# brantburnett/Snappier

Hardware: AMD Instinct MI355X
Metric: uncompressed GB/s block compress+decompress, 64 KiB blocks (higher is better)
Workload: dtype u8

## Files before the change

### snappier_amd/csrc/compress_lanes.hip

```cpp
#include <cstdlib>

#include "snp_device.h"

#ifndef SNP_CL_FLAT
#define SNP_CL_FLAT 1
#endif
#ifndef SNP_CL_SLOTS
#define SNP_CL_SLOTS 1
#endif

namespace {

constexpr u32 kDefaultSlots = SNP_CL_SLOTS;

constexpr u32 crc_step32(u32 x)
{
    for (int k = 0; k < 32; ++k) x = (x >> 1) ^ ((x & 1u) ? 0x82F63B78u : 0u);
    return x;
}

__device__ __forceinline__ u32 check_bits(u32 bytes) { return (bytes * 0x9E3779B1u) & 0xffff0000u; }

__device__ __forceinline__ u32 table_swap(u32* p, u32 v) { return __hip_atomic_exchange(p, v, __ATOMIC_RELAXED, __HIP_MEMORY_SCOPE_AGENT); }

struct LaneCtx {
    const u8* src;
    u8* dst;
    u32* table;
    u32 first4;
    u32 n;
    u32 mask;
    u32 hmask;
};

template <int VARIANT>
__device__ __forceinline__ u32 lane_hash(const LaneCtx& c, u32 bytes, const u16 (*lut)[256])
{
    u32 hash;
    if constexpr (VARIANT == SNP_HASH_CRC32C) {
        hash = lut[0][bytes & 0xffu] ^ lut[1][(bytes >> 8) & 0xffu] ^ lut[2][(bytes >> 16) & 0xffu] ^ lut[3][bytes >> 24] ^ c.hmask;
    } else {
        hash = (0x1e35a7bdu * bytes) >> 17;
    }
    return (hash & c.mask) >> 1;
}

__device__ __forceinline__ u32 lane_emit_literal(const LaneCtx& c, u32 op, u32 s, u32 len)
{
    u8* o = c.dst + op;
    const u32 k = len - 1;
    u32 hdr;
    if (k < 60) { o[0] = static_cast<u8>(k << 2); hdr = 1; }
    else if (k < 256) { o[0] = static_cast<u8>(60u << 2); o[1] = static_cast<u8>(k); hdr = 2; }
    else { o[0] = static_cast<u8>(61u << 2); o[1] = static_cast<u8>(k); o[2] = static_cast<u8>(k >> 8); hdr = 3; }
    const u8* src = c.src + s;
    u8* d = o + hdr;
    u32 i = 0;
    for (; i + 16 <= len; i += 16)
        *reinterpret_cast<snp_u128_unaligned*>(d + i) = *reinterpret_cast<const snp_u128_unaligned*>(src + i);
    for (; i + 4 <= len; i += 4) st32u(d + i, ld32u(src + i));
    for (; i < len; ++i) d[i] = src[i];
    return op + hdr + len;
}

__device__ __forceinline__ u32 lane_emit_literal16(const LaneCtx& c, u32 op, u32 s, u32 len, const snp_u128_unaligned& first, u32 cap, bool merge)
{
    u8* o = c.dst + op;
    const u32 k = len - 1;
    if (merge && len <= 15 && op + 16 <= cap) {
        snp_u128_unaligned w;
        w.v[0] = (first.v[0] << 8) | (k << 2);
        w.v[1] = __builtin_amdgcn_alignbit(first.v[1], first.v[0], 24);
        w.v[2] = __builtin_amdgcn_alignbit(first.v[2], first.v[1], 24);
        w.v[3] = __builtin_amdgcn_alignbit(first.v[3], first.v[2], 24);
        *reinterpret_cast<snp_u128_unaligned*>(o) = w;
        return op + 1 + len;
    }
    u32 hdr;
    if (k < 60) { o[0] = static_cast<u8>(k << 2); hdr = 1; }
    else if (k < 256) { o[0] = static_cast<u8>(60u << 2); o[1] = static_cast<u8>(k); hdr = 2; }
    else { o[0] = static_cast<u8>(61u << 2); o[1] = static_cast<u8>(k); o[2] = static_cast<u8>(k >> 8); hdr = 3; }
    u8* d = o + hdr;
    if (len >= 16 || op + hdr + 16 <= cap) {
        *reinterpret_cast<snp_u128_unaligned*>(d) = first;
    } else {
        u32 w[4] = {first.v[0], first.v[1], first.v[2], first.v[3]};
        u32 at = 0, wi = 0;
        if (len & 8) { st32u(d, w[0]); st32u(d + 4, w[1]); at = 8; wi = 2; }
        if (len & 4) { st32u(d + at, w[wi]); at += 4; ++wi; }
        u32 rest = w[wi & 3];
        if (len & 2) { d[at] = static_cast<u8>(rest); d[at + 1] = static_cast<u8>(rest >> 8); rest >>= 16; at += 2; }
        if (len & 1) d[at] = static_cast<u8>(rest);
    }
    if (len > 16) {
        const u8* src = c.src + s;
        u32 i = 16;
        for (; i + 16 <= len; i += 16)
            *reinterpret_cast<snp_u128_unaligned*>(d + i) = *reinterpret_cast<const snp_u128_unaligned*>(src + i);
        if (i < len)
            *reinterpret_cast<snp_u128_unaligned*>(d + len - 16) = *reinterpret_cast<const snp_u128_unaligned*>(src + len - 16);
    }
    return op + hdr + len;
}

__device__ __forceinline__ u32 lane_emit_copy64(u8* dst, u32 op, u32 off, u32 len, u32 cap)
{
    u8* o = dst + op;
    const bool one = len < 12 && off < 2048;
    const u32 w = one ? (1u | ((len - 4) << 2) | ((off >> 8) << 5) | ((off & 0xffu) << 8)) : (2u | ((len - 1) << 2) | (off << 8));
    if (op + 4 <= cap) {
        st32u(o, w);
    } else {
        o[0] = static_cast<u8>(w);
        o[1] = static_cast<u8>(w >> 8);
        if (!one) o[2] = static_cast<u8>(w >> 16);
    }
    return op + (one ? 2u : 3u);
}

__device__ __forceinline__ u32 lane_emit_copy(u8* dst, u32 op, u32 off, u32 len, u32 cap = 0)
{
    while (len >= 68) { op = lane_emit_copy64(dst, op, off, 64, cap); len -= 64; }
    if (len > 64) { op = lane_emit_copy64(dst, op, off, 60, cap); len -= 60; }
    return lane_emit_copy64(dst, op, off, len, cap);
}

__device__ __forceinline__ u32 lane_find_match_length(const u8* src, u32 s1, u32 s2, u32 n)
{
    u32 matched = 0;
    while (s2 + matched + 8 <= n) {
        const u64 x = ld64u(src + s1 + matched) ^ ld64u(src + s2 + matched);
        if (x) return matched + (static_cast<u32>(__builtin_ctzll(x)) >> 3);
        matched += 8;
    }
    while (s2 + matched < n && src[s1 + matched] == src[s2 + matched]) ++matched;
    return matched;
}

constexpr u32 kStageStride = 100;

struct OutStage {
    u8* lds;
    u32 flushed;
};

__device__ __forceinline__ void stage_flush64(const LaneCtx& c, OutStage& st)
{
    u8* g = c.dst + st.flushed;
    typedef u32 v4u __attribute__((ext_vector_type(4), aligned(1)));
#pragma unroll
    for (u32 i = 0; i < 64; i += 16) {
        const snp_u128_unaligned q = *reinterpret_cast<const snp_u128_unaligned*>(st.lds + i);
        const v4u v = {q.v[0], q.v[1], q.v[2], q.v[3]};
        __builtin_nontemporal_store(v, reinterpret_cast<v4u*>(g + i));
    }
    const snp_u128_unaligned t0 = *reinterpret_cast<const snp_u128_unaligned*>(st.lds + 64);
    const snp_u128_unaligned t1 = *reinterpret_cast<const snp_u128_unaligned*>(st.lds + 80);
    *reinterpret_cast<snp_u128_unaligned*>(st.lds) = t0;
    *reinterpret_cast<snp_u128_unaligned*>(st.lds + 16) = t1;
    st.flushed += 64;
}

__device__ __forceinline__ void stage_drain(const LaneCtx& c, OutStage& st, u32 op)
{
    const u32 fill = op - st.flushed;
    u8* g = c.dst + st.flushed;
    u32 i = 0;
    for (; i + 16 <= fill; i += 16)
        *reinterpret_cast<snp_u128_unaligned*>(g + i) = *reinterpret_cast<const snp_u128_unaligned*>(st.lds + i);
    for (; i < fill; ++i) g[i] = st.lds[i];
    st.flushed = op;
}

enum : int {
    kOptBlindLiterals = 1,
    kOptBlindLiteral16 = 2,
    kOptBlindCopies = 4,
    kOptShortExtend = 8,
    kOptStagedOutput = 16,
    kOptExchangeProbe = 64,
    kOptInputWindow = 128,
};

template <int VARIANT, u32 kSlots, bool SMALL>
__global__ __launch_bounds__(SNP_WAVE) void k_compress_lanes(const u8* __restrict__ in, const u64* __restrict__ in_off,
                                                            const u32* __restrict__ in_len, u32 nblocks,
                                                            u8* __restrict__ out, const u64* __restrict__ out_off,
                                                            u32* __restrict__ out_len, i32* __restrict__ status,
                                                            int emit_varint, const snp_table_pieces tp, int opts,
                                                            const u32* __restrict__ max_len, u32 small_max)
{
    __shared__ u16 lut[4][256];
    if (VARIANT == SNP_HASH_CRC32C) {
        for (u32 e = threadIdx.x; e < 1024; e += blockDim.x)
            lut[e >> 8][e & 255u] = static_cast<u16>(crc_step32((e & 255u) << (8 * (e >> 8))) & 0x7ffeu);
        __syncthreads();
    }
    __shared__ u8 s_out[SMALL ? 16 : SNP_WAVE * kStageStride];
    const u32 b = blockIdx.x * blockDim.x + threadIdx.x;
    const u32 maxlen = *max_len;
    if (SMALL ? maxlen > small_max : (small_max != 0 && maxlen <= small_max)) return;
    extern __shared__ __attribute__((aligned(16))) u8 s_dyn[];
    const u32 tstride = maxlen > 16384 ? 16384u : maxlen < 256 ? 256u : (2u << (31u - __clz(maxlen - 1)));
    u32* wt;
    {
        const u32 first = blockIdx.x * blockDim.x;
        const u32 mine = nblocks - first < blockDim.x ? nblocks - first : blockDim.x;
        const u32 piece = first / tp.piece_frags;
        wt = tp.p[piece] + static_cast<size_t>(first - piece * tp.piece_frags) * tstride;
        const size_t words = static_cast<size_t>(mine) * tstride;
        if (tstride == 16384u) {
            typedef u32 v4u __attribute__((ext_vector_type(4)));
            const v4u zero4 = {0, 0, 0, 0};
            for (size_t i = static_cast<size_t>(threadIdx.x) * 4; i < words; i += static_cast<size_t>(blockDim.x) * 4)
                __builtin_nontemporal_store(zero4, reinterpret_cast<v4u*>(wt + i));
        } else {
            for (size_t i = static_cast<size_t>(threadIdx.x) * 4; i < words; i += static_cast<size_t>(blockDim.x) * 4)
                *reinterpret_cast<uint4*>(wt + i) = make_uint4(0, 0, 0, 0);
        }
        asm volatile("s_waitcnt vmcnt(0)" ::: "memory");
    }
    if (b >= nblocks) return;
    const bool staged = (opts & kOptStagedOutput) != 0;
    const bool t_swap = kSlots == 1 && (opts & kOptExchangeProbe) != 0;
    bool in_win = (opts & kOptInputWindow) != 0;
    OutStage stg{(SMALL ? s_dyn + blockDim.x * (small_max + 16u) : s_out) + threadIdx.x * kStageStride, 0};

    LaneCtx c;
    c.dst = out + out_off[b];
    c.n = in_len[b];
    c.table = wt + static_cast<size_t>(threadIdx.x) * tstride;
    const u32 n = c.n;
    if constexpr (SMALL) {
        const u8* g = in + in_off[b];
        u8* mine = s_dyn + threadIdx.x * (small_max + 16u);
        u32 i = 0;
        for (; i + 16 <= n; i += 16) {
            const snp_u128_unaligned q = *reinterpret_cast<const snp_u128_unaligned*>(g + i);
            *reinterpret_cast<uint4*>(mine + i) = make_uint4(q.v[0], q.v[1], q.v[2], q.v[3]);
        }
        for (; i + 4 <= n; i += 4) *reinterpret_cast<u32*>(mine + i) = ld32u(g + i);
        for (; i < n; ++i) mine[i] = g[i];
        c.src = mine;
    } else {
        c.src = in + in_off[b];
    }
    c.first4 = n >= 4 ? ld32u(c.src) : 0u;
    if (n > SNP_BLOCK_SIZE) { out_len[b] = 0; status[b] = SNP_ERR_BAD_ARG; return; }

    u32 op = 0;
    if (emit_varint) {
        u32 v = n;
        while (v >= 128) { c.dst[op++] = static_cast<u8>(v | 0x80u); v >>= 7; }
        c.dst[op++] = static_cast<u8>(v);
    }
    stg.flushed = op;

    u32 ip = 0;
#if SNP_CL_FLAT
    enum : u32 { kScan = 0, kPost = 1, kExtend = 2, kDone = 3 };
    u32 mode = kDone;
    u32 next_emit = 0, skip = 32, cand = 0, base = 0, mlen = 0, limit = 0;
    snp_u128_unaligned win = {};
    u32 win_at = 0x80000000u;
    in_win = in_win && n >= 32;
    if (n >= 15) {
        const u32 tsize = n > 16384 ? 16384u : n < 256 ? 256u : (2u << (31u - __clz(n - 1)));
        c.mask = 2 * (tsize - 1);
        c.hmask = static_cast<u16>(crc_step32(c.mask) & 0x7ffeu);
        limit = n - 15;
        mode = kScan;
        ip = 1;
    }
    const u32 lit_cap = (opts & kOptBlindLiterals) ? 32u + n + n / 6u : 0u;
    while (__any(mode != kDone)) {
        u32 cp_len = 0, cp_off = 0;
        u32 lit_len = 0;
        snp_u128_unaligned lit16 = {};
        const bool post = mode == kPost;
        const bool scanning = mode == kScan || post;
        u32 p[kSlots], nx[kSlots], sk[kSlots], d[kSlots], h[kSlots], cv[kSlots];
        bool legal[kSlots];
        u64 w0 = 0;
        if (scanning) {
            u32 q = ip, sv = skip;
            bool ok = true;
#pragma unroll
            for (u32 k = 0; k < kSlots; ++k) {
                const u32 bb = post ? 0u : sv >> 5;
                sv += bb;
                p[k] = q;
                nx[k] = q + bb;
                sk[k] = sv;
                ok = ok && (post ? k == 0 : nx[k] <= limit);
                legal[k] = ok;
                q = nx[k];
            }
            const u32 at = ip - (post ? 1u : 0u);
            if (in_win) {
                u32 o = at - win_at;
                if (o > 8u) {
                    win_at = min(at, n - 16u);
                    win = *reinterpret_cast<const snp_u128_unaligned*>(c.src + win_at);
                    o = at - win_at;
                }
                const u32 dq = o >> 2, sh = (o & 3u) * 8u;
                const u32 a0 = dq == 0 ? win.v[0] : dq == 1 ? win.v[1] : win.v[2];
                const u32 a1 = dq == 0 ? win.v[1] : dq == 1 ? win.v[2] : win.v[3];
                const u32 a2 = dq == 0 ? win.v[2] : dq == 1 ? win.v[3] : 0u;
                const u64 lo = (static_cast<u64>(a1) << 32) | a0;
                w0 = sh ? (lo >> sh) | (static_cast<u64>(a2) << (64u - sh)) : lo;
            } else {
                w0 = ld64u(c.src + at);
            }
        } else {
#pragma unroll
            for (u32 k = 0; k < kSlots; ++k) { p[k] = nx[k] = sk[k] = 0; legal[k] = false; }
        }
        const bool ext = mode == kExtend;
        const bool ext_wide = ext && base + mlen + 32 <= n;
        snp_u128_unaligned xa0 = {}, xa1 = {}, xb0 = {}, xb1 = {};
        if (ext_wide) {
            const u8* a = c.src + cand + mlen;
            const u8* bq = c.src + base + mlen;
            xa0 = *reinterpret_cast<const snp_u128_unaligned*>(a);
            xb0 = *reinterpret_cast<const snp_u128_unaligned*>(bq);
            if (!(opts & kOptShortExtend)) {
                xa1 = *reinterpret_cast<const snp_u128_unaligned*>(a + 16);
                xb1 = *reinterpret_cast<const snp_u128_unaligned*>(bq + 16);
            }
        }
        u32 hm1 = ~0u, vm1 = 0;
        bool swapped = false;
        if (scanning) {
            if (post) {
                const u32 dm1 = static_cast<u32>(w0);
                hm1 = lane_hash<VARIANT>(c, dm1, lut);
                vm1 = (ip - 1) | check_bits(dm1);
                if (tstride == 16384u) __builtin_nontemporal_store(vm1, &c.table[hm1]);
                else c.table[hm1] = vm1;
                d[0] = static_cast<u32>(w0 >> 8);
            } else {
                d[0] = static_cast<u32>(w0);
            }
#pragma unroll
            for (u32 k = 1; k < kSlots; ++k) {
                d[k] = 0;
                if (legal[k]) {
                    const u32 delta = p[k] - p[0];
                    d[k] = delta <= 4 ? static_cast<u32>(w0 >> (8 * delta)) : ld32u(c.src + p[k]);
                }
            }
#pragma unroll
            for (u32 k = 0; k < kSlots; ++k) h[k] = lane_hash<VARIANT>(c, d[k], lut);
            if (t_swap) {
                swapped = legal[0] && h[0] != hm1;
                cv[0] = !legal[0] ? 0u : swapped ? table_swap(&c.table[h[0]], p[0] | check_bits(d[0])) : vm1;
            } else {
#pragma unroll
                for (u32 k = 0; k < kSlots; ++k) cv[k] = legal[k] ? c.table[h[k]] : 0u;
            }
        }
        if (ext) {
            bool finished = false;
            if (ext_wide) {
                const u64 x0 = (static_cast<u64>(xa0.v[0] ^ xb0.v[0])) | (static_cast<u64>(xa0.v[1] ^ xb0.v[1]) << 32);
                const u64 x1 = (static_cast<u64>(xa0.v[2] ^ xb0.v[2])) | (static_cast<u64>(xa0.v[3] ^ xb0.v[3]) << 32);
                const u64 x2 = (static_cast<u64>(xa1.v[0] ^ xb1.v[0])) | (static_cast<u64>(xa1.v[1] ^ xb1.v[1]) << 32);
                const u64 x3 = (static_cast<u64>(xa1.v[2] ^ xb1.v[2])) | (static_cast<u64>(xa1.v[3] ^ xb1.v[3]) << 32);
                finished = true;
                if (x0) mlen += static_cast<u32>(__builtin_ctzll(x0)) >> 3;
                else if (x1) mlen += 8 + (static_cast<u32>(__builtin_ctzll(x1)) >> 3);
                else if (opts & kOptShortExtend) { mlen += 16; finished = false; }
                else if (x2) mlen += 16 + (static_cast<u32>(__builtin_ctzll(x2)) >> 3);
                else if (x3) mlen += 24 + (static_cast<u32>(__builtin_ctzll(x3)) >> 3);
                else { mlen += 32; finished = false; }
            } else {
                for (u32 k = 0; k < 4 && !finished; ++k) {
                    if (base + mlen + 8 <= n) {
                        const u64 x = ld64u(c.src + cand + mlen) ^ ld64u(c.src + base + mlen);
                        if (x) { mlen += static_cast<u32>(__builtin_ctzll(x)) >> 3; finished = true; }
                        else mlen += 8;
                    } else {
                        while (base + mlen < n && c.src[cand + mlen] == c.src[base + mlen]) ++mlen;
                        finished = true;
                    }
                }
            }
            if (finished) {
                ip = base + mlen;
                cp_len = mlen;
                cp_off = base - cand;
                mode = ip >= limit ? kDone : kPost;
            }
        }
        if (scanning) {
#pragma unroll
            for (u32 k = 1; k < kSlots; ++k)
#pragma unroll
                for (u32 i = 0; i < k; ++i)
                    if (legal[k] && h[i] == h[k]) cv[k] = p[i] | check_bits(d[i]);
            u32 kw = kSlots;
#pragma unroll
            for (u32 k = kSlots; k-- > 0;) {
                const u32 pos = cv[k] & 0xffffu;
                const bool want = legal[k] && (pos == 0 ? c.first4 == d[k] : (cv[k] & 0xffff0000u) == check_bits(d[k]));
                if (want) kw = k;
            }
            u32 wp = 0, wpos = 0;
#pragma unroll
            for (u32 k = 0; k < kSlots; ++k)
                if (kw == k) { wp = p[k]; wpos = cv[k] & 0xffffu; }
            snp_u128_unaligned cb = {}, pb = {}, lb = {};
            if (kw < kSlots) {
                cb = *reinterpret_cast<const snp_u128_unaligned*>(c.src + wpos);
                pb = *reinterpret_cast<const snp_u128_unaligned*>(c.src + wp);
                if (!post) lb = *reinterpret_cast<const snp_u128_unaligned*>(c.src + next_emit);
            }
            bool ended = false;
#pragma unroll
            for (u32 k = 0; k < kSlots; ++k) {
                if (!ended && k <= kw) {
                    if (!legal[k]) {
                        if (!post) { ended = true; ip = next_emit; mode = kDone; }
                    } else if (!swapped) {
                        c.table[h[k]] = p[k] | check_bits(d[k]);
                    }
                }
            }
            if (!ended) {
                bool hit = false;
                if (kw < kSlots) {
                    const u64 x0 = (static_cast<u64>(cb.v[0] ^ pb.v[0])) | (static_cast<u64>(cb.v[1] ^ pb.v[1]) << 32);
                    const u64 x1 = (static_cast<u64>(cb.v[2] ^ pb.v[2])) | (static_cast<u64>(cb.v[3] ^ pb.v[3]) << 32);
                    hit = static_cast<u32>(x0) == 0;
                    if (hit) {
                        if (!post) {
                            if (staged) { lit_len = wp - next_emit; lit16 = lb; }
                            else op = lane_emit_literal16(c, op, next_emit, wp - next_emit, lb, lit_cap, (opts & kOptBlindLiteral16) != 0);
                        }
                        base = wp;
                        cand = wpos;
                        if (x0) mlen = static_cast<u32>(__builtin_ctzll(x0)) >> 3;
                        else if (x1) mlen = 8 + (static_cast<u32>(__builtin_ctzll(x1)) >> 3);
                        else mlen = 16;
                        if (mlen < 16) {
                            ip = base + mlen;
                            cp_len = mlen;
                            cp_off = base - cand;
                            mode = ip >= limit ? kDone : kPost;
                        } else {
                            mode = kExtend;
                        }
                    }
                }
                if (!hit) {
                    if (post) {
                        next_emit = ip;
                        ++ip;
                        skip = 32;
                        mode = kScan;
                    } else {
                        const u32 last = kw < kSlots ? kw : kSlots - 1;
#pragma unroll
                        for (u32 k = 0; k < kSlots; ++k)
                            if (k == last) { ip = nx[k]; skip = sk[k]; }
                    }
                }
            }
        }
        if (!staged) {
            if (cp_len) op = lane_emit_copy(c.dst, op, cp_off, cp_len, (opts & kOptBlindCopies) ? lit_cap : 0u);
        } else {
            if (lit_len) {
                if (lit_len <= 15) {
                    snp_u128_unaligned w;
                    w.v[0] = (lit16.v[0] << 8) | ((lit_len - 1) << 2);
                    w.v[1] = __builtin_amdgcn_alignbit(lit16.v[1], lit16.v[0], 24);
                    w.v[2] = __builtin_amdgcn_alignbit(lit16.v[2], lit16.v[1], 24);
                    w.v[3] = __builtin_amdgcn_alignbit(lit16.v[3], lit16.v[2], 24);
                    *reinterpret_cast<snp_u128_unaligned*>(stg.lds + (op - stg.flushed)) = w;
                    op += 1 + lit_len;
                } else {
                    stage_drain(c, stg, op);
                    op = lane_emit_literal16(c, op, next_emit, lit_len, lit16, 0u, false);
                    stg.flushed = op;
                }
            }
            u32 len = cp_len;
            while (len) {
                const u32 piece = len >= 68 ? 64u : len > 64 ? 60u : len;
                const bool one = piece < 12 && cp_off < 2048;
                const u32 w = one ? (1u | ((piece - 4) << 2) | ((cp_off >> 8) << 5) | ((cp_off & 0xffu) << 8))
                                  : (2u | ((piece - 1) << 2) | (cp_off << 8));
                st32u(stg.lds + (op - stg.flushed), w);
                op += one ? 2u : 3u;
                len -= piece;
                if (op - stg.flushed >= 64) stage_flush64(c, stg);
            }
            if (op - stg.flushed >= 64) stage_flush64(c, stg);
        }
    }
    if (staged) stage_drain(c, stg, op);
#else
    if (n >= 15) {
        const u32 tsize = n > 16384 ? 16384u : n < 256 ? 256u : (2u << (31u - __clz(n - 1)));
        c.mask = 2 * (tsize - 1);
        c.hmask = static_cast<u16>(crc_step32(c.mask) & 0x7ffeu);
        const u32 limit = n - 15;
        for (;;) {
            const u32 next_emit = ip;
            ++ip;
            u32 skip = 32;
            u32 cand;
            for (;;) {
                const u32 data = ld32u(c.src + ip);
                const u32 bb = skip >> 5;
                skip += bb;
                const u32 nxt = ip + bb;
                if (nxt > limit) { ip = next_emit; goto emit_remainder; }
                const u32 h = lane_hash<VARIANT>(c, data, lut);
                cand = c.table[h] & 0xffffu;
                c.table[h] = ip | check_bits(data);
                if (ld32u(c.src + cand) == data) break;
                ip = nxt;
            }
            op = lane_emit_literal(c, op, next_emit, ip - next_emit);
            for (;;) {
                const u32 base = ip;
                const u32 matched = 4 + lane_find_match_length(c.src, cand + 4, ip + 4, n);
                ip += matched;
                op = lane_emit_copy(c.dst, op, base - cand, matched);
                if (ip >= limit) goto emit_remainder;
                const u32 dm1 = ld32u(c.src + ip - 1);
                c.table[lane_hash<VARIANT>(c, dm1, lut)] = (ip - 1) | check_bits(dm1);
                const u32 data = ld32u(c.src + ip);
                const u32 h = lane_hash<VARIANT>(c, data, lut);
                cand = c.table[h] & 0xffffu;
                c.table[h] = ip | check_bits(data);
                if (ld32u(c.src + cand) != data) break;
            }
        }
    }
emit_remainder:
#endif
    if (ip < n) op = lane_emit_literal(c, op, ip, n - ip);
    out_len[b] = op;
    status[b] = SNP_OK;
}

}

namespace {
__global__ __launch_bounds__(SNP_WAVE) void k_probe_tables(const snp_table_pieces tp, u32 nblocks, u32 probes)
{
    const u32 g = blockIdx.x * SNP_WAVE + threadIdx.x;
    if (g >= nblocks) return;
    u32* t = tp.p[(g / tp.piece_frags) % tp.n] + static_cast<size_t>(g % tp.piece_frags) * 16384u;
    u32 st = g * 2654435761u + 1u;
    for (u32 i = 0; i < probes; ++i) {
        const u32 h = (st * 0x1e35a7bdu) >> 18;
        const u32 v = table_swap(&t[h], i);
        st = st * 1664525u + 1013904223u + v;
    }
    if (st == 0x12345678u) tp.p[0][0] = st;
}
}

extern "C" hipError_t snp_probe_tables(const snp_table_pieces* tp, u32 nblocks, u32 probes, hipStream_t stream, float* ms)
{
    hipEvent_t a, b;
    hipError_t e = hipEventCreate(&a);
    if (e != hipSuccess) return e;
    e = hipEventCreate(&b);
    if (e != hipSuccess) { (void)hipEventDestroy(a); return e; }
    const u32 grid = (nblocks + SNP_WAVE - 1) / SNP_WAVE;
    hipLaunchKernelGGL(k_probe_tables, dim3(grid), dim3(SNP_WAVE), 0, stream, *tp, nblocks, 64u);
    (void)hipEventRecord(a, stream);
    hipLaunchKernelGGL(k_probe_tables, dim3(grid), dim3(SNP_WAVE), 0, stream, *tp, nblocks, probes);
    (void)hipEventRecord(b, stream);
    e = hipEventSynchronize(b);
    if (e == hipSuccess) e = hipEventElapsedTime(ms, a, b);
    (void)hipEventDestroy(a);
    (void)hipEventDestroy(b);
    return e;
}

namespace {
__global__ void k_debug_lane_match_length(const u8* buf, u32 n, u32 s1, u32 s2, u32* out)
{
    if (threadIdx.x == 0) *out = lane_find_match_length(buf, s1, s2, n);
}
}
extern "C" int snp_debug_lane_match_length(const u8* d_buf, u32 n, u32 s1, u32 s2, u32* d_out, hipStream_t stream)
{
    hipLaunchKernelGGL(k_debug_lane_match_length, dim3(1), dim3(SNP_WAVE), 0, stream, d_buf, n, s1, s2, d_out);
    return static_cast<int>(hipGetLastError());
}

extern "C" size_t snp_compress_lanes_workspace(u32 nblocks) { return static_cast<size_t>(nblocks) * 16384u * sizeof(u32); }

__global__ __launch_bounds__(256) void k_max_len(const u32* __restrict__ in_len, u32 nblocks, u32* __restrict__ max_len)
{
    u32 m = 0;
    for (u32 i = blockIdx.x * 256 + threadIdx.x; i < nblocks; i += gridDim.x * 256) m = max(m, in_len[i]);
    for (int sh = 32; sh >= 1; sh >>= 1) m = max(m, static_cast<u32>(__shfl_xor(static_cast<int>(m), sh, 64)));
    if ((threadIdx.x & 63u) == 0) atomicMax(max_len, m);
}

extern "C" hipError_t snp_launch_compress_lanes(const u8* in, const u64* in_off, const u32* in_len, u32 nblocks, u8* out,
                                                const u64* out_off, u32* out_len, i32* status, int variant,
                                                int emit_varint, const snp_table_pieces* tables, u32* max_len, hipStream_t stream, const snp_lane_tuning* tune)
{
    if (nblocks == 0) return hipSuccess;
    hipError_t e = snp_zero_words_async(max_len, 1, stream);
    if (e != hipSuccess) return e;
    const u32 mgrid = (nblocks + 255) / 256 < 1024 ? (nblocks + 255) / 256 : 1024u;
    hipLaunchKernelGGL(k_max_len, dim3(mgrid), dim3(256), 0, stream, in_len, nblocks, max_len);
    const char* env = SNP_GETENV("SNAPPIER_HIP_LANES_PER_WAVE");
    const bool two_probes = (tune->hint & 256) != 0;
    const u32 small_hint = ((static_cast<u32>(tune->hint) >> 9) & 63u) << 4;
    const u32 lanes_hint = tune->lanes_per_wave ? static_cast<u32>(tune->lanes_per_wave) : static_cast<u32>(tune->hint & 255);
    u32 per = env ? static_cast<u32>(atoi(env)) : lanes_hint ? lanes_hint : (nblocks >= 131072 ? 64u : nblocks >= 8192 ? 32u : 16u);
    if (per != 64 && per != 32 && per != 16 && per != 8) per = 64;
    const u32 grid = (nblocks + per - 1) / per;
    const char* ex = SNP_GETENV("SNAPPIER_HIP_EXACT_LITERALS");
    const char* oe = SNP_GETENV("SNAPPIER_HIP_CL_OPTS");
    const int opts = ((ex && ex[0] == '1') ? 0 : oe ? (atoi(oe) & 255) : tune->opts >= 0 ? (tune->opts & 255)
                      : ((nblocks >= 32768 ? 23 : 7) | 64 | ((nblocks >= 131072 && !two_probes) ? 128 : 0)));
    const char* se = SNP_GETENV("SNAPPIER_HIP_CL_SLOTS");
    const u32 slots = se ? static_cast<u32>(atoi(se)) : tune->probes > 0 ? static_cast<u32>(tune->probes) : ((nblocks >= 131072 && !two_probes) ? kDefaultSlots : 2u);
    const char* sm = SNP_GETENV("SNAPPIER_HIP_CL_SMALL");
    u32 small_max = sm ? (static_cast<u32>(atoi(sm)) + 15u) & ~15u : tune->small_bytes >= 0 ? (static_cast<u32>(tune->small_bytes) + 15u) & ~15u : small_hint;
    if (small_max > 2048) small_max = 0;
    if (small_max) {
        const char* sp = SNP_GETENV("SNAPPIER_HIP_CL_SMALL_PER");
        u32 sper = sp ? static_cast<u32>(atoi(sp)) : tune->small_lanes ? static_cast<u32>(tune->small_lanes) : 32u;
        if (sper != 64 && sper != 32 && sper != 16) sper = 32;
        const u32 sgrid = (nblocks + sper - 1) / sper;
        const u32 dyn = sper * (small_max + 16u + kStageStride);
        bool small_ok = true;
#define SNP_LAUNCH_SMALL(V)                                                                                                                         \
    do {                                                                                                                                            \
        if (dyn > 48u * 1024u && hipFuncSetAttribute(reinterpret_cast<const void*>(&k_compress_lanes<V, 2, true>), hipFuncAttributeMaxDynamicSharedMemorySize, static_cast<int>(dyn)) != hipSuccess) { \
            small_ok = false;                                                                                                                       \
            break;                                                                                                                                  \
        }                                                                                                                                           \
        hipLaunchKernelGGL((k_compress_lanes<V, 2, true>), dim3(sgrid), dim3(sper), dyn, stream, in, in_off, in_len, nblocks, out, out_off, out_len, status, \
                           emit_varint, *tables, opts, max_len, small_max);                                                                    \
        small_ok = hipGetLastError() == hipSuccess;                                                                                                 \
    } while (0)
        if (variant == SNP_HASH_CRC32C) SNP_LAUNCH_SMALL(SNP_HASH_CRC32C); else SNP_LAUNCH_SMALL(SNP_HASH_MUL);
#undef SNP_LAUNCH_SMALL
        if (!small_ok) {
            (void)hipGetLastError();
            small_max = 0;
        }
    }
#define SNP_LAUNCH_CL(V, S)                                                                                          \
    hipLaunchKernelGGL((k_compress_lanes<V, S, false>), dim3(grid), dim3(per), 0, stream, in, in_off, in_len, nblocks, out,    \
                       out_off, out_len, status, emit_varint, *tables, opts, max_len, small_max)
    if (variant == SNP_HASH_CRC32C) { if (slots == 1) SNP_LAUNCH_CL(SNP_HASH_CRC32C, 1); else if (slots >= 4) SNP_LAUNCH_CL(SNP_HASH_CRC32C, 4); else if (slots == 3) SNP_LAUNCH_CL(SNP_HASH_CRC32C, 3); else SNP_LAUNCH_CL(SNP_HASH_CRC32C, 2); }
    else { if (slots == 1) SNP_LAUNCH_CL(SNP_HASH_MUL, 1); else if (slots >= 4) SNP_LAUNCH_CL(SNP_HASH_MUL, 4); else if (slots == 3) SNP_LAUNCH_CL(SNP_HASH_MUL, 3); else SNP_LAUNCH_CL(SNP_HASH_MUL, 2); }
#undef SNP_LAUNCH_CL
    return hipGetLastError();
}
```

Measured before the change: 98.95.

## Add opt-in explicit step-machine compress loop with split issue/consume phases

Adds an alternative per-lane compression loop, selected by a new option bit and only for the single-slot launch. It splits each trip into issue and consume phases separated by explicit waitcnt barriers, so loads from divergent lanes (input window, table probe, candidate compare, extend) are issued together and their latency overlaps across the wave. The shared emit and window-extract code is factored into helpers reused by the existing loop. The path is off unless the new option is passed, and the hard waitcnt(0) barriers may serialise more than the compiler's own scheduling.

```diff
diff --git a/snappier_amd/csrc/compress_lanes.hip b/snappier_amd/csrc/compress_lanes.hip
--- a/snappier_amd/csrc/compress_lanes.hip
+++ b/snappier_amd/csrc/compress_lanes.hip
@@ -178,11 +178,252 @@
     kOptBlindCopies = 4,
     kOptShortExtend = 8,
     kOptStagedOutput = 16,
+    kOptStepMachine = 32,
     kOptExchangeProbe = 64,
     kOptInputWindow = 128,
 };
 
-template <int VARIANT, u32 kSlots, bool SMALL>
+__device__ __forceinline__ u32 lane_emit_trip(const LaneCtx& c, OutStage& stg, u32 op, bool staged, int opts, u32 lit_cap, u32 next_emit,
+                                              u32 lit_len, const snp_u128_unaligned& lit16, u32 cp_len, u32 cp_off)
+{
+    if (!staged) {
+        if (cp_len) op = lane_emit_copy(c.dst, op, cp_off, cp_len, (opts & kOptBlindCopies) ? lit_cap : 0u);
+    } else {
+        if (lit_len) {
+            if (lit_len <= 15) {
+                snp_u128_unaligned w;
+                w.v[0] = (lit16.v[0] << 8) | ((lit_len - 1) << 2);
+                w.v[1] = __builtin_amdgcn_alignbit(lit16.v[1], lit16.v[0], 24);
+                w.v[2] = __builtin_amdgcn_alignbit(lit16.v[2], lit16.v[1], 24);
+                w.v[3] = __builtin_amdgcn_alignbit(lit16.v[3], lit16.v[2], 24);
+                *reinterpret_cast<snp_u128_unaligned*>(stg.lds + (op - stg.flushed)) = w;
+                op += 1 + lit_len;
+            } else {
+                stage_drain(c, stg, op);
+                op = lane_emit_literal16(c, op, next_emit, lit_len, lit16, 0u, false);
+                stg.flushed = op;
+            }
+        }
+        u32 len = cp_len;
+        while (len) {
+            const u32 piece = len >= 68 ? 64u : len > 64 ? 60u : len;
+            const bool one = piece < 12 && cp_off < 2048;
+            const u32 w = one ? (1u | ((piece - 4) << 2) | ((cp_off >> 8) << 5) | ((cp_off & 0xffu) << 8))
+                              : (2u | ((piece - 1) << 2) | (cp_off << 8));
+            st32u(stg.lds + (op - stg.flushed), w);
+            op += one ? 2u : 3u;
+            len -= piece;
+            if (op - stg.flushed >= 64) stage_flush64(c, stg);
+        }
+        if (op - stg.flushed >= 64) stage_flush64(c, stg);
+    }
+    return op;
+}
+
+__device__ __forceinline__ u64 window_bytes8(u32 v0, u32 v1, u32 v2, u32 v3, u32 o)
+{
+    const u32 dq = o >> 2, sh = (o & 3u) * 8u;
+    const u32 a0 = dq == 0 ? v0 : dq == 1 ? v1 : v2;
+    const u32 a1 = dq == 0 ? v1 : dq == 1 ? v2 : v3;
+    const u32 a2 = dq == 0 ? v2 : dq == 1 ? v3 : 0u;
+    const u64 lo = (static_cast<u64>(a1) << 32) | a0;
+    return sh ? (lo >> sh) | (static_cast<u64>(a2) << (64u - sh)) : lo;
+}
+
+enum : u32 { sInput = 0, sTable = 1, sCand = 2, sExtend = 3, sDone = 4 };
+
+template <int VARIANT>
+__device__ __forceinline__ u32 lane_step_loop(const LaneCtx& c, OutStage& stg, const u16 (*lut)[256], int opts, bool nt_table, bool in_win, u32 op, u32& ip_out)
+{
+    const u32 n = c.n;
+    const bool staged = (opts & kOptStagedOutput) != 0;
+    const bool t_swap = (opts & kOptExchangeProbe) != 0;
+    const u32 lit_cap = (opts & kOptBlindLiterals) ? 32u + n + n / 6u : 0u;
+    const u32 limit = n - 15;
+    const u32 cover = in_win ? 8u : 0u;
+    u32 ip = 0, next_emit = 0, skip = 32, cand = 0, base = 0, mlen = 0, cv = 0, st = sDone;
+    bool post = false;
+    snp_u128_unaligned win = {};
+    u32 win_at = 0x80000000u;
+    snp_u128_unaligned q0 = {}, q1 = {}, q2 = {}, q3 = {};
+    u32 d = 0;
+    u64 w8 = 0;
+    auto begin_probe = [&]() {
+        if (!post && ip + (skip >> 5) > limit) { ip = next_emit; st = sDone; return; }
+        st = (ip - (post ? 1u : 0u)) - win_at > cover ? sInput : sTable;
+    };
+    auto finish_copy = [&](u32& cp_len, u32& cp_off) {
+        ip = base + mlen;
+        cp_len = mlen;
+        cp_off = base - cand;
+        if (ip >= limit) { st = sDone; return; }
+        post = true;
+        begin_probe();
+    };
+    auto issue_input = [&]() {
+        const u32 at = ip - (post ? 1u : 0u);
+        if (in_win) {
+            win_at = min(at, n - 16u);
+            win = *reinterpret_cast<const snp_u128_unaligned*>(c.src + win_at);
+        } else {
+            win_at = at;
+            w8 = ld64u(c.src + at);
+        }
+    };
+    auto consume_input = [&]() {
+        if (!in_win) { win.v[0] = static_cast<u32>(w8); win.v[1] = static_cast<u32>(w8 >> 32); }
+        st = sTable;
+    };
+    auto wait_all = [&]() {
+        asm volatile("" ::: "memory");
+        __builtin_amdgcn_s_waitcnt(0x0F70);
+        asm volatile("" ::: "memory");
+    };
+    if (n >= 15) {
+        ip = 1;
+        begin_probe();
+    }
+    while (__any(st != sDone)) {
+        u32 cp_len = 0, cp_off = 0, lit_len = 0;
+        snp_u128_unaligned lit16 = {};
+        if (st == sInput) {
+            issue_input();
+        } else if (st == sTable) {
+            const u64 w0 = window_bytes8(win.v[0], win.v[1], win.v[2], win.v[3], ip - (post ? 1u : 0u) - win_at);
+            u32 hm1 = ~0u, vm1 = 0;
+            if (post) {
+                const u32 dm1 = static_cast<u32>(w0);
+                hm1 = lane_hash<VARIANT>(c, dm1, lut);
+                vm1 = (ip - 1) | check_bits(dm1);
+                d = static_cast<u32>(w0 >> 8);
+            } else {
+                d = static_cast<u32>(w0);
+            }
+            const u32 h = lane_hash<VARIANT>(c, d, lut);
+            const u32 mine = ip | check_bits(d);
+            if (h == hm1) {
+                cv = vm1;
+                c.table[h] = mine;
+            } else {
+                if (post) {
+                    if (nt_table) __builtin_nontemporal_store(vm1, &c.table[hm1]);
+                    else c.table[hm1] = vm1;
+                }
+                if (t_swap) {
+                    cv = table_swap(&c.table[h], mine);
+                } else {
+                    cv = c.table[h];
+                    c.table[h] = mine;
+                }
+            }
+        } else if (st == sExtend) {
+            if (base + mlen + 32 <= n) {
+                const u8* a = c.src + cand + mlen;
+                const u8* bq = c.src + base + mlen;
+                q0 = *reinterpret_cast<const snp_u128_unaligned*>(a);
+                q1 = *reinterpret_cast<const snp_u128_unaligned*>(bq);
+                if (!(opts & kOptShortExtend)) {
+                    q2 = *reinterpret_cast<const snp_u128_unaligned*>(a + 16);
+                    q3 = *reinterpret_cast<const snp_u128_unaligned*>(bq + 16);
+                }
+            }
+        }
+        wait_all();
+        if (st == sInput) {
+            consume_input();
+        } else if (st == sTable) {
+            const u32 pos = cv & 0xffffu;
+            if (pos == 0 ? c.first4 == d : (cv & 0xffff0000u) == check_bits(d)) {
+                st = sCand;
+            } else if (post) {
+                next_emit = ip;
+                ++ip;
+                skip = 32;
+                post = false;
+                begin_probe();
+            } else {
+                const u32 bb = skip >> 5;
+                ip += bb;
+                skip += bb;
+                begin_probe();
+            }
+        } else if (st == sExtend) {
+            bool finished = false;
+            if (base + mlen + 32 <= n) {
+                const u64 x0 = (static_cast<u64>(q0.v[0] ^ q1.v[0])) | (static_cast<u64>(q0.v[1] ^ q1.v[1]) << 32);
+                const u64 x1 = (static_cast<u64>(q0.v[2] ^ q1.v[2])) | (static_cast<u64>(q0.v[3] ^ q1.v[3]) << 32);
+                const u64 x2 = (static_cast<u64>(q2.v[0] ^ q3.v[0])) | (static_cast<u64>(q2.v[1] ^ q3.v[1]) << 32);
+                const u64 x3 = (static_cast<u64>(q2.v[2] ^ q3.v[2])) | (static_cast<u64>(q2.v[3] ^ q3.v[3]) << 32);
+                finished = true;
+                if (x0) mlen += static_cast<u32>(__builtin_ctzll(x0)) >> 3;
+                else if (x1) mlen += 8 + (static_cast<u32>(__builtin_ctzll(x1)) >> 3);
+                else if (opts & kOptShortExtend) { mlen += 16; finished = false; }
+                else if (x2) mlen += 16 + (static_cast<u32>(__builtin_ctzll(x2)) >> 3);
+                else if (x3) mlen += 24 + (static_cast<u32>(__builtin_ctzll(x3)) >> 3);
+                else { mlen += 32; finished = false; }
+            } else {
+                for (u32 k = 0; k < 4 && !finished; ++k) {
+                    if (base + mlen + 8 <= n) {
+                        const u64 x = ld64u(c.src + cand + mlen) ^ ld64u(c.src + base + mlen);
+                        if (x) { mlen += static_cast<u32>(__builtin_ctzll(x)) >> 3; finished = true; }
+                        else mlen += 8;
+                    } else {
+                        while (base + mlen < n && c.src[cand + mlen] == c.src[base + mlen]) ++mlen;
+                        finished = true;
+                    }
+                }
+            }
+            if (finished) finish_copy(cp_len, cp_off);
+        }
+        if (st == sCand) {
+            q0 = *reinterpret_cast<const snp_u128_unaligned*>(c.src + (cv & 0xffffu));
+            q1 = *reinterpret_cast<const snp_u128_unaligned*>(c.src + ip);
+            if (!post) q2 = *reinterpret_cast<const snp_u128_unaligned*>(c.src + next_emit);
+        } else if (st == sInput) {
+            issue_input();
+        }
+        wait_all();
+        if (st == sCand) {
+            const u64 x0 = (static_cast<u64>(q0.v[0] ^ q1.v[0])) | (static_cast<u64>(q0.v[1] ^ q1.v[1]) << 32);
+            const u64 x1 = (static_cast<u64>(q0.v[2] ^ q1.v[2])) | (static_cast<u64>(q0.v[3] ^ q1.v[3]) << 32);
+            if (static_cast<u32>(x0) == 0) {
+                if (!post) {
+                    if (staged) { lit_len = ip - next_emit; lit16 = q2; }
+                    else op = lane_emit_literal16(c, op, next_emit, ip - next_emit, q2, lit_cap, (opts & kOptBlindLiteral16) != 0);
+                }
+                base = ip;
+                cand = cv & 0xffffu;
+                if (x0) mlen = static_cast<u32>(__builtin_ctzll(x0)) >> 3;
+                else if (x1) mlen = 8 + (static_cast<u32>(__builtin_ctzll(x1)) >> 3);
+                else mlen = 16;
+                if (mlen < 16) {
+                    if (in_win) { win = q1; win_at = base; }
+                    finish_copy(cp_len, cp_off);
+                } else {
+                    st = sExtend;
+                }
+            } else if (post) {
+                next_emit = ip;
+                ++ip;
+                skip = 32;
+                post = false;
+                begin_probe();
+            } else {
+                const u32 bb = skip >> 5;
+                ip += bb;
+                skip += bb;
+                begin_probe();
+            }
+        } else if (st == sInput) {
+            consume_input();
+        }
+        op = lane_emit_trip(c, stg, op, staged, opts, lit_cap, next_emit, lit_len, lit16, cp_len, cp_off);
+    }
+    ip_out = ip;
+    return op;
+}
+
+template <int VARIANT, u32 kSlots, bool SMALL, bool STEPS = false>
 __global__ __launch_bounds__(SNP_WAVE) void k_compress_lanes(const u8* __restrict__ in, const u64* __restrict__ in_off,
                                                             const u32* __restrict__ in_len, u32 nblocks,
                                                             u8* __restrict__ out, const u64* __restrict__ out_off,
@@ -190,6 +431,7 @@
                                                             int emit_varint, const snp_table_pieces tp, int opts,
                                                             const u32* __restrict__ max_len, u32 small_max)
 {
+    static_assert(!STEPS || (kSlots == 1 && !SMALL), "the step machine is a form of the one-probe-per-trip general launch");
     __shared__ u16 lut[4][256];
     if (VARIANT == SNP_HASH_CRC32C) {
         for (u32 e = threadIdx.x; e < 1024; e += blockDim.x)
@@ -272,6 +514,10 @@
         mode = kScan;
         ip = 1;
     }
+    if constexpr (STEPS) {
+        op = lane_step_loop<VARIANT>(c, stg, lut, opts, tstride == 16384u, in_win, op, ip);
+        mode = kDone;
+    }
     const u32 lit_cap = (opts & kOptBlindLiterals) ? 32u + n + n / 6u : 0u;
     while (__any(mode != kDone)) {
         u32 cp_len = 0, cp_off = 0;
@@ -304,12 +550,7 @@
                     win = *reinterpret_cast<const snp_u128_unaligned*>(c.src + win_at);
                     o = at - win_at;
                 }
-                const u32 dq = o >> 2, sh = (o & 3u) * 8u;
-                const u32 a0 = dq == 0 ? win.v[0] : dq == 1 ? win.v[1] : win.v[2];
-                const u32 a1 = dq == 0 ? win.v[1] : dq == 1 ? win.v[2] : win.v[3];
-                const u32 a2 = dq == 0 ? win.v[2] : dq == 1 ? win.v[3] : 0u;
-                const u64 lo = (static_cast<u64>(a1) << 32) | a0;
-                w0 = sh ? (lo >> sh) | (static_cast<u64>(a2) << (64u - sh)) : lo;
+                w0 = window_bytes8(win.v[0], win.v[1], win.v[2], win.v[3], o);
             } else {
                 w0 = ld64u(c.src + at);
             }
@@ -469,37 +710,7 @@
                 }
             }
         }
-        if (!staged) {
-            if (cp_len) op = lane_emit_copy(c.dst, op, cp_off, cp_len, (opts & kOptBlindCopies) ? lit_cap : 0u);
-        } else {
-            if (lit_len) {
-                if (lit_len <= 15) {
-                    snp_u128_unaligned w;
-                    w.v[0] = (lit16.v[0] << 8) | ((lit_len - 1) << 2);
-                    w.v[1] = __builtin_amdgcn_alignbit(lit16.v[1], lit16.v[0], 24);
-                    w.v[2] = __builtin_amdgcn_alignbit(lit16.v[2], lit16.v[1], 24);
-                    w.v[3] = __builtin_amdgcn_alignbit(lit16.v[3], lit16.v[2], 24);
-                    *reinterpret_cast<snp_u128_unaligned*>(stg.lds + (op - stg.flushed)) = w;
-                    op += 1 + lit_len;
-                } else {
-                    stage_drain(c, stg, op);
-                    op = lane_emit_literal16(c, op, next_emit, lit_len, lit16, 0u, false);
-                    stg.flushed = op;
-                }
-            }
-            u32 len = cp_len;
-            while (len) {
-                const u32 piece = len >= 68 ? 64u : len > 64 ? 60u : len;
-                const bool one = piece < 12 && cp_off < 2048;
-                const u32 w = one ? (1u | ((piece - 4) << 2) | ((cp_off >> 8) << 5) | ((cp_off & 0xffu) << 8))
-                                  : (2u | ((piece - 1) << 2) | (cp_off << 8));
-                st32u(stg.lds + (op - stg.flushed), w);
-                op += one ? 2u : 3u;
-                len -= piece;
-                if (op - stg.flushed >= 64) stage_flush64(c, stg);
-            }
-            if (op - stg.flushed >= 64) stage_flush64(c, stg);
-        }
+        op = lane_emit_trip(c, stg, op, staged, opts, lit_cap, next_emit, lit_len, lit16, cp_len, cp_off);
     }
     if (staged) stage_drain(c, stg, op);
 #else
@@ -657,11 +868,12 @@
             small_max = 0;
         }
     }
-#define SNP_LAUNCH_CL(V, S)                                                                                          \
-    hipLaunchKernelGGL((k_compress_lanes<V, S, false>), dim3(grid), dim3(per), 0, stream, in, in_off, in_len, nblocks, out,    \
+#define SNP_LAUNCH_CL(V, S, ...)                                                                                     \
+    hipLaunchKernelGGL((k_compress_lanes<V, S, false, ##__VA_ARGS__>), dim3(grid), dim3(per), 0, stream, in, in_off, in_len, nblocks, out,    \
                        out_off, out_len, status, emit_varint, *tables, opts, max_len, small_max)
-    if (variant == SNP_HASH_CRC32C) { if (slots == 1) SNP_LAUNCH_CL(SNP_HASH_CRC32C, 1); else if (slots >= 4) SNP_LAUNCH_CL(SNP_HASH_CRC32C, 4); else if (slots == 3) SNP_LAUNCH_CL(SNP_HASH_CRC32C, 3); else SNP_LAUNCH_CL(SNP_HASH_CRC32C, 2); }
-    else { if (slots == 1) SNP_LAUNCH_CL(SNP_HASH_MUL, 1); else if (slots >= 4) SNP_LAUNCH_CL(SNP_HASH_MUL, 4); else if (slots == 3) SNP_LAUNCH_CL(SNP_HASH_MUL, 3); else SNP_LAUNCH_CL(SNP_HASH_MUL, 2); }
+    const bool steps = slots == 1 && (opts & kOptStepMachine) != 0;
+    if (variant == SNP_HASH_CRC32C) { if (steps) SNP_LAUNCH_CL(SNP_HASH_CRC32C, 1, true); else if (slots == 1) SNP_LAUNCH_CL(SNP_HASH_CRC32C, 1); else if (slots >= 4) SNP_LAUNCH_CL(SNP_HASH_CRC32C, 4); else if (slots == 3) SNP_LAUNCH_CL(SNP_HASH_CRC32C, 3); else SNP_LAUNCH_CL(SNP_HASH_CRC32C, 2); }
+    else { if (steps) SNP_LAUNCH_CL(SNP_HASH_MUL, 1, true); else if (slots == 1) SNP_LAUNCH_CL(SNP_HASH_MUL, 1); else if (slots >= 4) SNP_LAUNCH_CL(SNP_HASH_MUL, 4); else if (slots == 3) SNP_LAUNCH_CL(SNP_HASH_MUL, 3); else SNP_LAUNCH_CL(SNP_HASH_MUL, 2); }
 #undef SNP_LAUNCH_CL
     return hipGetLastError();
 }
```

Result: slower. 93.40 (-5.6%).
